# KMS-TEAM/vi_slam

Measured on AMD Instinct MI355X. Metric: frames/sec ORB extract+match, higher is better.
Workload: dtype u8; 1 GPU; kitti00_mono_1241x376_n1000; nfeatures=1000, nlevels=8, contexts_in_flight=4, distinct_frames=32, match=SearchForInitialization(prev frame) window 100

## Files before the change

### vi_slam_amd/csrc/vslam_host.cpp

```cpp
#include "vslam_host.h"
#include "vslam_undistort.h"
#include "vslam_frustum.h"
#include "vslam_kb8.h"
#include "vslam_two_view.h"
#include "vslam_matchdev.h"

#include <algorithm>
#include <climits>
#include <cmath>
#include <cstdlib>
#include <cstring>

namespace vslam {

static inline int cv_round(float v) { return (int)lrintf(v); }
static inline int cv_round(double v) { return (int)lrint(v); }
static inline int cv_floor(float v) {
    int i = (int)v;
    return i - (i > v);
}
static inline int cv_ceil(float v) {
    int i = (int)v;
    return i + (i < v);
}
static inline int16_t sat_short(float v) {
    int iv = cv_round(v);
    return (int16_t)std::min(std::max(iv, (int)SHRT_MIN), (int)SHRT_MAX);
}

void build_tables(int nfeatures, float scaleFactorF, int nlevels, ExtractorTables& t) {
    const double scaleFactor = scaleFactorF;
    t.nlevels = nlevels;
    t.scale.assign(nlevels, 1.0f);
    t.sigma2.assign(nlevels, 1.0f);
    for (int i = 1; i < nlevels; i++) {
        t.scale[i] = (float)(t.scale[i - 1] * scaleFactor);
        t.sigma2[i] = t.scale[i] * t.scale[i];
    }
// ... 585 lines not shown
        P.nIni[l] = nIni;
        P.hX[l] = (float)W / nIni;
        P.selOff[l] = selOff;
        const int cap_l = std::max(P.N[l] + 3, 4 * nIni) + 1;
        selOff += cap_l;
        maxNodes = std::max(maxNodes, cap_l);
        maxNodes = std::max(maxNodes, (cell_first[l + 1] - cell_first[l] + 1 + 3) / 4);
        if (nIni > 64) fits = false;
    }
    P.selStride = selOff;
    P.maxNodes = (maxNodes + 15) & ~15;
    const size_t nb = (node_bytes(P.maxNodes) + 15) & ~(size_t)15;
    int maxcells = 0;
    for (int l = 0; l < L; l++) {
        const int W = lw[l] - 2 * VSLAM_FAST_BORDER, H = P.H[l], nIni = P.nIni[l];
        int D = 1;
        while ((nIni << (2 * D)) < P.N[l]) D++;
        D += 1;
        if (forced_depth >= 0) D = forced_depth;
        D = std::max(1, std::min(D, 11));
        while (D > 1 && (((long long)nIni << (2 * D)) > 16384 || nb + 2 * (((size_t)nIni << (2 * D)) + 1) * 4 + 16 > budget))
            D--;
        P.fineD[l] = D;
        maxcells = std::max(maxcells, nIni << (2 * D));
        std::vector<uint32_t> xs, ys;
        build_oct_lut(W, H, D, xs, ys);
        P.lutOff[l] = (int32_t)P.lut.size();
        P.lutW[l] = (int32_t)xs.size();
        P.lut.insert(P.lut.end(), xs.begin(), xs.end());
        P.lut.insert(P.lut.end(), ys.begin(), ys.end());
    }
    P.fineLdsOff = (int32_t)nb;
    P.fineLdsBytes = (int32_t)(2 * ((size_t)maxcells + 1) * 4 + 16);
    P.fits = fits && nb + (size_t)P.fineLdsBytes <= 160 * 1024 && node_bytes(P.maxNodes) <= 150 * 1024;
}

void build_oct_lut(int W, int H, int D, std::vector<uint32_t>& xs, std::vector<uint32_t>& ys) {
    const int nIni = (int)std::round((float)W / (float)H);
    const float hX = (float)W / (float)nIni;
    xs.assign((size_t)W + 1, 0u);
    ys.assign((size_t)H + 1, 0u);
    for (int x = 0; x <= W; x++) {
        int b = (int)((float)x / hX);
        b = std::min(b, nIni - 1);
        int x0 = (int)(hX * (float)b), x1 = (int)(hX * (float)(b + 1));
        uint32_t code = 0;
        for (int d = 0; d < D; d++) {
            const int mx = x0 + ((x1 - x0 + 1) >> 1);
            const int q = x < mx ? 0 : 1;
            code = (code << 2) | (uint32_t)q;
            if (q) x0 = mx; else x1 = mx;
        }
        xs[x] = ((uint32_t)b << (2 * D)) | code;
    }
    for (int y = 0; y <= H; y++) {
        int y0 = 0, y1 = H;
        uint32_t code = 0;
        for (int d = 0; d < D; d++) {
            const int my = y0 + ((y1 - y0 + 1) >> 1);
            const int q = y < my ? 0 : 1;
            code = (code << 2) | ((uint32_t)q << 1);
            if (q) y0 = my; else y1 = my;
        }
        ys[y] = code;
    }
}

// ... 489 lines not shown
                cur[p] = t.in ? 1 : 0;
            }
            score = vslam_tv::report_score(score);
            if (scores) scores[it] = score;
            const vslam_tv::Best was = best;
            best = vslam_tv::best_take(best, score, it);
            if (best.index != was.index && mask && used) memcpy(mask, cur.data(), (size_t)used);
        }
        (model ? R.best_f : R.best_h) = best.index;
        (model ? R.score_f : R.score_h) = best.index >= 0 ? best.score : 0.0f;
    }
    return err ? VSLAM_ERR_INVALID : n > cap ? VSLAM_ERR_UNSUPPORTED : VSLAM_OK;
}

uint64_t vslamh_layout(uint64_t align, const uint64_t* sizes, int n, uint64_t* off) {
    std::vector<size_t> s(sizes, sizes + n), o(n);
    const size_t total = vslam::layout_parts((size_t)align, s.data(), n, o.data());
    for (int i = 0; i < n; i++) off[i] = o[i];
    return total;
}

int vslamh_oct_lut_check(int W, int H, int D) {
    std::vector<uint32_t> xs, ys;
    vslam::build_oct_lut(W, H, D, xs, ys);
    int bad = 0;
    for (int y = 0; y <= H; y++)
        for (int x = 0; x <= W; x++) bad += (xs[x] | ys[y]) != vslam::oct_key_path(x, y, W, H, D);
    return bad;
}
unsigned vslamh_oct_key_path(int x, int y, int W, int H, int depth) { return vslam::oct_key_path(x, y, W, H, depth); }

int vslamh_keypoint_capacity(const int* quota, const int* lw, const int* lh, int nlevels, int nfeatures) {
    return vslam::keypoint_capacity(quota, lw, lh, nlevels, nfeatures);
}

int vslamh_oct_plan(const int* quota, const int* lw, const int* lh, const int* cell_first, int nlevels, int forced_depth,
                    int budget, int node_per, int node_fixed, int32_t* ctx6, int32_t* lvl4) {
    vslam::OctPlan P;
    vslam::plan_octree(quota, lw, lh, cell_first, nlevels, forced_depth, (size_t)budget,
                       [=](int n) { return (size_t)n * node_per + node_fixed; }, P);
    int bad = 0;
    for (int l = 0; l < nlevels; l++) {
        const int W = P.lutW[l] - 1, H = P.H[l];
        const uint32_t *xs = P.lut.data() + P.lutOff[l], *ys = xs + P.lutW[l];
        for (int y = 0; y <= H; y++)
            for (int x = 0; x <= W; x++) bad += (xs[x] | ys[y]) != vslam::oct_key_path(x, y, W, H, P.fineD[l]);
        const int32_t o[4] = {P.nIni[l], P.selOff[l], P.fineD[l], P.lutW[l]};
        memcpy(lvl4 + 4 * l, o, sizeof(o));
    }
    const int32_t c[6] = {P.maxNodes, P.selStride, P.fineLdsOff, P.fineLdsBytes, P.fits, bad};
    memcpy(ctx6, c, sizeof(c));
    return 0;
}

int vslamh_band_tables(const uint16_t* cells5, int ncells, int nlevels, int max_cells, int max_width, uint32_t* words4,
                       int cap_bands, uint8_t* classes, int cap_class_bytes, int32_t* info5) {
    static_assert(sizeof(vslam::HostCell) == 10 && sizeof(vslam::BandWords) == 16, "rows of five u16 / four u32");
    const vslam::HostCell* c = (const vslam::HostCell*)cells5;
    std::vector<vslam::HostBand> b;
    vslam::build_bands(std::vector<vslam::HostCell>(c, c + ncells), max_cells, max_width, b);
    vslam::BandTables T;
    vslam::pack_bands(b, nlevels, T);
    if ((int)b.size() > cap_bands || (int)T.classes.size() > cap_class_bytes) return -1;
    memcpy(words4, T.bands.data(), T.bands.size() * sizeof(vslam::BandWords));
    memcpy(classes, T.classes.data(), T.classes.size());
    const int32_t o[5] = {(int32_t)(T.classes.size() / 272), T.max_wh, T.max_iw, T.max_cells, T.ok};
// ... 350 lines not shown
```

### vi_slam_amd/csrc/vslam_init_kernel.hip

```cpp
#include "vslam_kernels.h"
#include "vslam_wave.h"
#include "vslam_matchdev.h"

#define SI_TH_LOW 50
#define SI_QPB_MAX 32

struct SiCand {
    float x, y, angle;
    uint16_t cell;
    uint16_t idx;
};
struct SiCandL {
    float x, y;
    uint32_t c;
    uint16_t cell;
    uint16_t idx;
};
struct SiQuery {
    float px, py, angle;
    uint32_t idx;
};

__host__ __device__ inline size_t si_pair_bytes(int max_c2, int M) {
    return 16 + (size_t)max_c2 * (sizeof(SiCand) + sizeof(SiQuery) + 4 * (size_t)M);
}

__global__ void __launch_bounds__(256)
k_si_topm(InitJobs jobs, int cap, SiBounds bnd, int window, int max_c2, int M, uint8_t* scratch, int SI_QPB) {
    extern __shared__ __align__(16) uint8_t sism[];
    SiCandL* cand = (SiCandL*)sism;
    uint32_t* wkeys = (uint32_t*)(cand + max_c2);
    SiCandL* tmpc = (SiCandL*)wkeys;
    __shared__ SiQuery s_q[SI_QPB_MAX];
    __shared__ int s_wcnt[4];
    __shared__ int s_col[SI_GRID_COLS + 1];
// ... 208 lines not shown
    return true;
}

#ifndef SIR_NT
#define SIR_NT 256
#endif
#define SIR_PEND 1u
#define SIR_ACC 2u
#define SIR_SCAN 4u
template <int MAXM>
__global__ void __launch_bounds__(SIR_NT)
k_si_replay(InitJobs jobs, int cap, SiBounds bnd, int window, float nnratio, int checkOri,
            int32_t* matches_out , float* prev_out ,
            int32_t* nmatch_out , int max_c2, int M, const uint8_t* scratch, int* fallbacks, int keys_lds_bytes) {
    extern __shared__ __align__(16) uint8_t sism[];
    const InitJob jb = jobs.job[blockIdx.x];
    const int tid = threadIdx.x, lane = tid & 63;
    const int n1 = min(*jb.cnt1, cap);
    const uint8_t* sp = scratch + (size_t)blockIdx.x * si_pair_bytes(max_c2, M);
    const int32_t* hdr = (const int32_t*)sp;
    const SiCand* gcand = (const SiCand*)(sp + 16);
    const SiQuery* gqry = (const SiQuery*)(gcand + max_c2);
    const uint32_t* topm = (const uint32_t*)(gqry + max_c2);
    const int c1 = hdr[0], c2 = hdr[1];
    uint4* slotlog = (uint4*)sism;
    int32_t* lister0 = (int32_t*)(slotlog + max_c2);
    int32_t* lister1 = lister0 + max_c2;
    uint32_t* kfirst = (uint32_t*)(lister1 + max_c2);
    uint32_t* ksecond = kfirst + max_c2;
    uint32_t* alog = ksecond + max_c2;
    int32_t* m12 = (int32_t*)(alog + max_c2);
    uint8_t* qstate = (uint8_t*)(m12 + cap);
    uint8_t* rotBin = qstate + max_c2;
    uint32_t* keys_lds = (uint32_t*)(sism + (((size_t)max_c2 * 37 + (size_t)cap * 5 + 15) & ~(size_t)15));
    const bool keys_in_lds = (size_t)c1 * M * 4 <= (size_t)keys_lds_bytes;
    const uint32_t* keysrc = keys_in_lds ? keys_lds : topm;
    if (keys_in_lds)
        for (int i = tid; i < c1 * M; i += SIR_NT) keys_lds[i] = topm[i];
    __shared__ int s_hist[VSLAM_HISTO_LENGTH];
    __shared__ int s_minpend[2], s_minwild[2], s_scanq, s_nlog, s_cnt;

    int32_t* mo = matches_out + (size_t)blockIdx.x * cap;
    float* po = prev_out + (size_t)blockIdx.x * cap * 2;
    const SiGridInv inv = si_grid_inv(bnd);
    const float r = (float)window;

    for (int c = tid; c < c2; c += SIR_NT) {
        slotlog[c] = make_uint4(0xFFFFFFFFu, 0xFFFFFFFFu, 0xFFFFFFFFu, 0xFFFFFFFFu);
        lister0[c] = 0x7FFFFFFF;
        lister1[c] = 0x7FFFFFFF;
    }
    for (int q = tid; q < c1; q += SIR_NT) qstate[q] = (uint8_t)SIR_PEND;
    for (int i = tid; i < n1; i += SIR_NT) {
        m12[i] = -1;
        rotBin[i] = 255;
    }
    if (tid < VSLAM_HISTO_LENGTH) s_hist[tid] = 0;
    if (tid == 0) {
        s_minpend[0] = s_minpend[1] = 0x7FFFFFFF;
        s_minwild[0] = s_minwild[1] = 0x7FFFFFFF;
        s_scanq = -1;
        s_nlog = 0;
        s_cnt = 0;
    }
    __syncthreads();

    int nfb = 0, nrounds = 0;
    for (int par = 0;; par ^= 1) {
        int32_t* lister = par ? lister1 : lister0;
        if (tid == 0) s_scanq = -1;
        for (int q = tid; q < c1; q += SIR_NT) {
            if (!(qstate[q] & SIR_PEND)) continue;
            uint32_t key[MAXM];
#pragma unroll
            for (int j = 0; j < MAXM; j++) key[j] = j < M ? keysrc[(size_t)q * M + j] : 0xFFFFFFFFu;
            int nvalid = 0;
            uint32_t gBest = 0xFFFFFFFFu, k2 = 0xFFFFFFFFu, klast = 0u;
#pragma unroll
            for (int j = 0; j < MAXM; j++) {
                if (j < M && key[j] != 0xFFFFFFFFu) {
                    nvalid++;
                    klast = key[j];
                    const uint32_t slot = si_key_index(key[j]), d = si_key_dist(key[j]);
                    if (!(sir_od_eff(slotlog[slot], (uint32_t)q) <= d)) {
                        if (d <= SI_TH_LOW) atomicMin(&lister[slot], q);
                        if (gBest == 0xFFFFFFFFu) gBest = key[j];
                        else if (k2 == 0xFFFFFFFFu) k2 = key[j];
                    }
                }
            }
            const bool full = nvalid == M;
            const uint32_t dlast = si_key_dist(klast);
            const bool wild = full && dlast <= SI_TH_LOW;
            bool accept = false, scan = false;
            if (gBest == 0xFFFFFFFFu) {
                scan = wild;
            } else if (si_key_dist(gBest) <= SI_TH_LOW) {
                uint32_t bestDist2 = k2 == 0xFFFFFFFFu ? 0x7FFFFFFFu : si_key_dist(k2);
                if (k2 == 0xFFFFFFFFu && full) {
                    if ((float)(int)si_key_dist(gBest) < __fmul_rn((float)(int)dlast, nnratio)) bestDist2 = dlast;
                    else scan = true;
                }
                if (!scan) accept = (float)(int)si_key_dist(gBest) < __fmul_rn((float)(int)bestDist2, nnratio);
            }
            kfirst[q] = gBest;
            ksecond[q] = k2;
// ... 91 lines not shown
            const int i = i0 + u * SIR_NT;
            m[u] = i < n1 ? m12[i] : -1;
        }
#pragma unroll
        for (int u = 0; u < 4; u++) {
            const int i = i0 + u * SIR_NT;
            o[u] = make_float2(0.0f, 0.0f);
            if (i < n1) {
                if (m[u] >= 0) o[u] = make_float2(jb.k2[m[u]].x, jb.k2[m[u]].y);
                else if (jb.prev) o[u] = make_float2(jb.prev[2 * i], jb.prev[2 * i + 1]);
                else o[u] = make_float2(jb.k1[i].x, jb.k1[i].y);
            }
        }
#pragma unroll
        for (int u = 0; u < 4; u++) {
            const int i = i0 + u * SIR_NT;
            if (i < n1) {
                mo[i] = m[u];
                po[2 * i] = o[u].x;
                po[2 * i + 1] = o[u].y;
                cnt += m[u] >= 0;
            }
        }
    }
#pragma unroll
    for (int o = 32; o > 0; o >>= 1) cnt += __shfl_xor(cnt, o, 64);
    if (lane == 0 && cnt) atomicAdd(&s_cnt, cnt);
    __syncthreads();
    if (tid == 0) nmatch_out[blockIdx.x] = hdr[2] ? -1 : s_cnt;
}

size_t vk_search_init_scratch_bytes(int npairs, int max_c2, int M) { return (size_t)npairs * si_pair_bytes(max_c2, M); }

static size_t si_topm_lds(int max_c2) { return (size_t)max_c2 * (sizeof(SiCand) + 4 * 4); }
static size_t si_replay_keys_lds(int max_c2, int M) {
    const size_t want = (size_t)max_c2 * M * 4;
    return want <= (64u << 10) ? want : 0;
}
static size_t si_replay_lds(int cap, int max_c2, int M = 0) {
    return (((size_t)max_c2 * 37 + (size_t)cap * 5 + 15) & ~(size_t)15) + si_replay_keys_lds(max_c2, M) + 16;
}

size_t vk_search_init_lds(int cap, int max_c2) { return std::max(si_topm_lds(max_c2), si_replay_lds(cap, max_c2)); }

int vk_search_init_set_max_lds(size_t bytes) {
    int rc = (int)hipFuncSetAttribute((const void*)k_si_topm, hipFuncAttributeMaxDynamicSharedMemorySize, (int)bytes);
    if (rc) return rc;
    rc = (int)hipFuncSetAttribute((const void*)k_si_replay<8>, hipFuncAttributeMaxDynamicSharedMemorySize, (int)bytes);
    if (rc) return rc;
    return (int)hipFuncSetAttribute((const void*)k_si_replay<SI_MAX_M>, hipFuncAttributeMaxDynamicSharedMemorySize, (int)bytes);
}

void vk_search_init(hipStream_t st, const InitJobs& jobs, int npairs, int cap, const SiBounds& bounds, int window,
                    float nnratio, int checkOri, int32_t* matches_out, float* prev_out, int32_t* nmatch_out,
                    int max_c2, int M, uint8_t* scratch, int* fallbacks, const vslam_tuning& T) {
    if (npairs <= 0) return;
    const int qv = T.si_queries_per_block;
    const int qpb = (qv == 8 || qv == 16 || qv == 32) ? qv : 16;
    const int chunks = (max_c2 + qpb - 1) / qpb;
    hipLaunchKernelGGL(k_si_topm, dim3(chunks, npairs), dim3(256), si_topm_lds(max_c2), st, jobs, cap, bounds,
                       window, max_c2, M, scratch, qpb);
    int keys_lds = (int)si_replay_keys_lds(max_c2, M);
    if (si_replay_lds(cap, max_c2, M) > (150u << 10)) keys_lds = 0;
    const size_t rlds = keys_lds ? si_replay_lds(cap, max_c2, M) : si_replay_lds(cap, max_c2);
    if (M <= 8)
        hipLaunchKernelGGL(k_si_replay<8>, dim3(npairs), dim3(SIR_NT), rlds, st, jobs, cap, bounds,
                           window, nnratio, checkOri, matches_out, prev_out, nmatch_out, max_c2, M, scratch, fallbacks, keys_lds);
    else
        hipLaunchKernelGGL(k_si_replay<SI_MAX_M>, dim3(npairs), dim3(SIR_NT), rlds, st, jobs, cap, bounds,
                           window, nnratio, checkOri, matches_out, prev_out, nmatch_out, max_c2, M, scratch, fallbacks, keys_lds);
}
```

### vi_slam_amd/csrc/vslam_octree_kernel.hip

```cpp
#include "vslam_kernels.h"

#include <mutex>

#ifndef O4BATCH
#define O4BATCH 8
#endif
typedef unsigned long long u64;

struct ONode {
    int16_t x0, y0, x1, y1;
    uint32_t begin;
    uint32_t cf;
};
#define ND_NOMORE(nd) ((nd).cf & 1u)

#define FB 21
#define FMASK ((1ull << FB) - 1)
__device__ __forceinline__ unsigned long long onehot(int q) { return q < 3 ? 1ull << (FB * q) : 0ull; }
__device__ __forceinline__ uint32_t fld(unsigned long long v, int q) { return (uint32_t)((v >> (FB * q)) & FMASK); }
__device__ __forceinline__ uint32_t nchildren(unsigned long long c, uint32_t count) {
    const uint32_t c0 = fld(c, 0), c1 = fld(c, 1), c2 = fld(c, 2);
    return (c0 != 0) + (c1 != 0) + (c2 != 0) + (count - c0 - c1 - c2 != 0);
}

template <typename T, int NT>
__device__ __forceinline__ T block_excl_scan(T v, T* s_wave, T* total) {
    const int tid = threadIdx.x, lane = tid & 63, wv = tid >> 6;
    T inc = v;
#pragma unroll
    for (int o = 1; o < 64; o <<= 1) {
        const T t = __shfl_up(inc, o, 64);
        if (lane >= o) inc += t;
    }
// ... 24 lines not shown
        const int mx = x0 + ((x1 - x0 + 1) >> 1), my = y0 + ((y1 - y0 + 1) >> 1);
        const int qx = x < mx ? 0 : 1, qy = y < my ? 0 : 1;
        code = (code << 2) | (uint32_t)qx | ((uint32_t)qy << 1);
        if (qx) x0 = mx; else x1 = mx;
        if (qy) y0 = my; else y1 = my;
    }
    return ((uint32_t)b << (2 * depth)) | code;
}

__device__ __forceinline__ uint32_t wave_incl_add(uint32_t v) {
#pragma unroll
    for (int o = 1; o < 64; o <<= 1) {
        const uint32_t t = __shfl_up(v, o, 64);
        if ((int)(threadIdx.x & 63) >= o) v += t;
    }
    return v;
}

__device__ __forceinline__ u64 deep_child_counts(const uint2* sorted, const uint32_t* PS, uint32_t path, int depth, int D,
                                                 float hX, int nIni, int Hh) {
    u64 c = 0ull;
    const uint32_t f = path >> (2 * (depth - D));
    for (uint32_t j = PS[f]; j < PS[f + 1]; j++) {
        const uint32_t kp = oct_key_path(sorted[j].x, hX, nIni, Hh, depth + 1);
        if ((kp >> 2) == path) c += onehot((int)(kp & 3u));
    }
    return c;
}

#define OCT_BEST(key, pos) ((((key) >> 24) << 20) | (0xFFFFFu - (uint32_t)(pos)))
#define OCT_BEST_POS(b) (0xFFFFFu - ((b) & 0xFFFFFu))

template <int OTV>
__global__ void __launch_bounds__(OTV)
k_octree_v4(const uint8_t* __restrict__ cand_region, size_t cand_stride, int ncells, OctParams P, uint32_t* keys_a,
            uint2* sorted_a, size_t pts_stride, uint32_t* sel_xyr, int32_t* sel_cnt, int32_t* err_flag,
            int32_t* deep_flags) {
    extern __shared__ __align__(16) uint8_t osm[];
    const int MAXN = P.maxNodes;
    ONode* cur = (ONode*)osm;
    ONode* nxt = cur + MAXN;
    uint32_t* Kq = (uint32_t*)(nxt + MAXN);
    u64* Cnt = (u64*)(nxt + MAXN) + MAXN;
    uint16_t* cb = (uint16_t*)(Cnt + MAXN);
    uint16_t* newIdx = cb + MAXN;
    uint16_t* prank = newIdx + MAXN;
    uint16_t* ordv = prank + MAXN;
    __shared__ uint32_t s_w32[OTV / 64];
    __shared__ int s_size, s_M, s_nexp, s_cut, s_deep;

    const int tid = threadIdx.x, lane = tid & 63, wv = tid >> 6;
    const int level = blockIdx.y, slot = blockIdx.x;
    const int N = P.N[level];
    const uint32_t* hdr = (const uint32_t*)(cand_region + (size_t)slot * cand_stride);
    const CellOut* cout = (const CellOut*)(hdr + 2);
    const uint32_t* cand = (const uint32_t*)(cout + ncells);
    uint32_t* pa = keys_a + (size_t)slot * pts_stride;
    uint2* sorted = sorted_a + (size_t)slot * pts_stride;
    uint32_t* out = sel_xyr + (size_t)slot * P.selStride + P.selOff[level];
    int32_t* ocnt = sel_cnt + slot * VSLAM_MAX_LEVELS + level;
    if (tid == 0) {
        deep_flags[slot * VSLAM_MAX_LEVELS + level] = 0;
        s_deep = 0;
    }
#ifdef VSLAM_OCT_STAMPS
    int dbgn3 = 0;
    unsigned long long* DBG3 = (unsigned long long*)P.dbg;
#ifndef VSLAM_OCT_STAMP_LEVEL
#define VSLAM_OCT_STAMP_LEVEL 0
#endif
#define STAMP3() do { if (DBG3 && tid == 0 && level == VSLAM_OCT_STAMP_LEVEL && slot == 0 && dbgn3 < 60) DBG3[dbgn3++] = __builtin_amdgcn_s_memrealtime(); } while (0)
#else
#define STAMP3() do { } while (0)
#endif
    STAMP3();

    const int c0 = P.cellFirst[level], c1 = P.cellFirst[level + 1];
    uint32_t off0 = 0;
    if (c0 > 0) {
        uint32_t before = 0;
        for (int c = tid; c < c0; c += OTV) before += cout[c].count;
        uint32_t tot;
        block_excl_scan<uint32_t, OTV>(before, s_w32, &tot);
        off0 = tot;
    }
    const int ncl = c1 - c0, K = (ncl + OTV - 1) / OTV;
    uint32_t mine = 0;
    for (int k = 0; k < K; k++) {
        const int c = c0 + tid * K + k;
        if (c < c1) mine += cout[c].count;
    }
    uint32_t ntot;
    uint32_t woff = block_excl_scan<uint32_t, OTV>(mine, s_w32, &ntot);
    const int n = (int)ntot;
    if (off0 + ntot > (uint32_t)P.ptsCap || n >= (1 << 20) || hdr[1] != 0) {
        if (tid == 0) {
// ... 91 lines not shown
            const uint32_t inc = wave_incl_add(h);
            if (c < cells) PS[c] = carry + inc - h;
            carry += (uint32_t)__builtin_amdgcn_readlane((int)inc, 63);
        }
        if (lane == 0) s_w32[wv] = carry;
        __syncthreads();
        uint32_t wo = 0;
        for (int k = 0; k < wv; k++) wo += s_w32[k];
        if (wo)
            for (int t = wv * tpw; t < t1; t++) {
                const int c = t * 64 + lane;
                if (c < cells) PS[c] += wo;
            }
        if (tid == 0) PS[cells] = (uint32_t)n;
    }
    __syncthreads();
    STAMP3();

    if (tid == 0) {
        int li = 0;
        for (int b = 0; b < nIni; b++) {
            const uint32_t cb0 = PS[(b + 1) << (2 * D)] - PS[b << (2 * D)];
            if (cb0) {
                ONode nd;
                nd.x0 = (int16_t)(int)__fmul_rn(hX, (float)b);
                nd.x1 = (int16_t)(int)__fmul_rn(hX, (float)(b + 1));
                nd.y0 = 0;
                nd.y1 = (int16_t)Hh;
                nd.begin = (uint32_t)b;
                nd.cf = (cb0 << 1) | (cb0 == 1 ? 1u : 0u);
                cur[li++] = nd;
            }
        }
        s_size = li;
    }
    __syncthreads();
    STAMP3();

    int phase = 1;
    bool haveSorted = false;
    const int KN = (MAXN + OTV - 1) / OTV;
    for (int iter = 0; iter < P.maxIter; iter++) {
        const int size0 = s_size;
        for (int k = 0; k < KN; k++) {
            const int v = tid * KN + k;
            if (v < size0) {
                const ONode nd = cur[v];
                u64 c = 0ull;
                uint32_t kq = 0u;
                if (!ND_NOMORE(nd)) {
                    const int depth = ND4_DEPTH(nd);
                    const uint32_t path = nd.begin;
                    if (depth < D) {
                        const uint32_t cb0 = path << (2 * (D - depth)), q4 = 1u << (2 * (D - depth - 1));
                        const uint32_t p0 = PS[cb0], p1 = PS[cb0 + q4], p2 = PS[cb0 + 2 * q4], p3 = PS[cb0 + 3 * q4];
                        c = (u64)(p1 - p0) | ((u64)(p2 - p1) << FB) | ((u64)(p3 - p2) << (2 * FB));
                    } else {
                        s_deep = 1;
                        if (haveSorted) c = deep_child_counts(sorted, PS, path, depth, D, hX, nIni, Hh);
                    }
                    kq = (ND4_COUNT(nd) << 12) | (uint32_t)(4095 - v);
                }
                Cnt[v] = c;
                Kq[v] = kq;
            }
        }
        if (tid < 4 && size0 + tid < ((size0 + 3) & ~3)) Kq[size0 + tid] = 0u;
        __syncthreads();
        if (s_deep && !haveSorted) {
            for (int i = tid; i < cells; i += OTV) Bst[i] = 0u;
            __syncthreads();
            for (int base = tid; base < n; base += O4BATCH * OTV) {
                uint32_t kk[O4BATCH], ff[O4BATCH];
#pragma unroll
                for (int j = 0; j < O4BATCH; j++) kk[j] = base + j * OTV < n ? pa[base + j * OTV] : 0u;
#pragma unroll
                for (int j = 0; j < O4BATCH; j++) ff[j] = base + j * OTV < n ? xs[kk[j] & 0xFFF] | ys[(kk[j] >> 12) & 0xFFF] : 0u;
#pragma unroll
                for (int j = 0; j < O4BATCH; j++) {
                    const int i = base + j * OTV;
                    if (i < n) sorted[PS[ff[j]] + atomicAdd(&Bst[ff[j]], 1u)] = make_uint2(kk[j], (uint32_t)i);
                }
            }
            haveSorted = true;
            __syncthreads();
            for (int k = 0; k < KN; k++) {
                const int v = tid * KN + k;
                if (v < size0) {
                    const ONode nd = cur[v];
                    if (!ND_NOMORE(nd) && ND4_DEPTH(nd) >= D)
                        Cnt[v] = deep_child_counts(sorted, PS, nd.begin, ND4_DEPTH(nd), D, hX, nIni, Hh);
                }
            }
            __syncthreads();
        }
        uint32_t nexp_mine = 0;
        for (int k = 0; k < KN; k++) {
            const int v = tid * KN + k;
            if (v < size0 && !ND_NOMORE(cur[v])) nexp_mine++;
        }
        uint32_t nexp;
        uint32_t rbase = block_excl_scan<uint32_t, OTV>(nexp_mine, s_w32, &nexp);
// ... 7 lines not shown
                    rbase++;
                }
            }
        } else {
            const uint4* K4 = (const uint4*)Kq;
            const int n4 = (size0 + 3) >> 2;
            for (int k = 0; k < KN; k++) {
                const int v = tid * KN + k;
                if (v < size0 && !ND_NOMORE(cur[v])) {
                    const uint32_t kv = Kq[v];
                    uint32_t r = 0;
#pragma unroll 4
                    for (int u = 0; u < n4; u++) {
                        const uint4 q = K4[u];
                        r += (q.x > kv) + (q.y > kv) + (q.z > kv) + (q.w > kv);
                    }
                    prank[v] = (uint16_t)r;
                    ordv[r] = (uint16_t)v;
                }
            }
        }
        __syncthreads();
        const int KE = ((int)nexp + OTV - 1) / OTV;
        uint32_t chl = 0;
        for (int k = 0; k < KE; k++) {
            const int r = tid * KE + k;
            if (r < (int)nexp) {
                const int v = ordv[r];
                chl += nchildren(Cnt[v], ND4_COUNT(cur[v]));
            }
        }
        uint32_t chtot;
        uint32_t chbase = block_excl_scan<uint32_t, OTV>(chl, s_w32, &chtot);
        if (tid == 0) s_cut = (int)nexp;
        __syncthreads();
        {
            uint32_t cb_run = chbase;
            for (int k = 0; k < KE; k++) {
                const int r = tid * KE + k;
                if (r < (int)nexp) {
                    const int v = ordv[r];
                    const uint32_t nch = nchildren(Cnt[v], ND4_COUNT(cur[v]));
                    if (phase == 2 && size0 + (int)cb_run - r >= N) atomicMin(&s_cut, r);
                    cb[v] = (uint16_t)cb_run;
                    cb_run += nch;
                }
            }
        }
        __syncthreads();
        const int ncut = s_cut;
        if (tid == 0) {
            int M;
            if (ncut >= (int)nexp) M = (int)chtot;
            else M = cb[ordv[ncut]];
            s_M = M;
            s_size = size0 + M - ncut;
            s_nexp = 0;
        }
        __syncthreads();
        const int M = s_M;
        uint32_t sv = 0;
        for (int k = 0; k < KN; k++) {
            const int v = tid * KN + k;
            if (v < size0) {
                const bool processed = !ND_NOMORE(cur[v]) && prank[v] < ncut;
                if (!processed) sv++;
            }
        }
        uint32_t svtot;
        uint32_t svbase = block_excl_scan<uint32_t, OTV>(sv, s_w32, &svtot);
        int nexp_children = 0;
        for (int k = 0; k < KN; k++) {
            const int v = tid * KN + k;
            if (v >= size0) continue;
            const ONode nd = cur[v];
            const bool processed = !ND_NOMORE(nd) && prank[v] < ncut;
            if (!processed) {
                nxt[M + svbase] = nd;
                svbase++;
            } else {
                const u64 c = Cnt[v];
                const int mx = nd.x0 + ((nd.x1 - nd.x0 + 1) >> 1), my = nd.y0 + ((nd.y1 - nd.y0 + 1) >> 1);
                const uint32_t depth1 = (uint32_t)ND4_DEPTH(nd) + 1u;
                int kq = 0;
                const int first = M - 1 - (int)cb[v];
                const uint32_t c3 = ND4_COUNT(nd) - fld(c, 0) - fld(c, 1) - fld(c, 2);
                for (int q = 0; q < 4; q++) {
                    const uint32_t cq = q < 3 ? fld(c, q) : c3;
                    if (!cq) continue;
                    ONode ch;
                    ch.x0 = (q & 1) ? (int16_t)mx : nd.x0;
                    ch.x1 = (q & 1) ? nd.x1 : (int16_t)mx;
                    ch.y0 = (q & 2) ? (int16_t)my : nd.y0;
                    ch.y1 = (q & 2) ? nd.y1 : (int16_t)my;
                    ch.begin = (nd.begin << 2) | (uint32_t)q;
                    ch.cf = (depth1 << 28) | (cq << 1) | (cq == 1 ? 1u : 0u);
                    nxt[first - kq] = ch;
                    if (cq > 1) nexp_children++;
                    kq++;
                }
            }
        }
        if (nexp_children) atomicAdd(&s_nexp, nexp_children);
        __syncthreads();
        { ONode* t = cur; cur = nxt; nxt = t; }
        const int size = s_size, nToExpand = s_nexp;
        __syncthreads();
        STAMP3();
        if (size >= N || size == size0) break;
        if (phase == 1 && size + nToExpand * 3 > N) phase = 2;
    }

    STAMP3();
    const int size = s_size;
    if (!haveSorted) {
        uint32_t* win = (uint32_t*)nxt;
        for (int v0 = 0; v0 < size; v0 += OTV / 4) {
            const int v = v0 + (tid >> 2), sub = tid & 3;
            uint32_t best = 0u;
            if (v < size) {
                const ONode nd = cur[v];
                const int sh = 2 * (D - ND4_DEPTH(nd));
                const uint32_t lo = nd.begin << sh, hi = (nd.begin + 1u) << sh;
                for (uint32_t j = lo + (uint32_t)sub; j < hi; j += 4) best = max(best, Bst[j]);
            }
            best = max(best, (uint32_t)__shfl_xor((int)best, 1, 64));
            best = max(best, (uint32_t)__shfl_xor((int)best, 2, 64));
            if (v < size && sub == 0) win[v] = OCT_BEST_POS(best);
        }
        __syncthreads();
        for (int v = tid; v < size; v += OTV) out[v] = pa[win[v]];
    } else {
        for (int v0 = 0; v0 < size; v0 += OTV / 4) {
            const int v = v0 + (tid >> 2), sub = tid & 3;
            u64 best = 0ull;
            uint32_t bkey = 0u;
            if (v < size) {
                const ONode nd = cur[v];
                const int depth = ND4_DEPTH(nd);
                const uint32_t path = nd.begin;
                if (depth <= D) {
                    const uint32_t lo = PS[path << (2 * (D - depth))], hi = PS[(path + 1u) << (2 * (D - depth))];
                    for (uint32_t j0 = lo + (uint32_t)sub; j0 < hi; j0 += 16) {
                        uint2 r[4];
#pragma unroll
                        for (int u = 0; u < 4; u++) r[u] = j0 + 4 * u < hi ? sorted[j0 + 4 * u] : make_uint2(0u, 0xFFFFFFFFu);
#pragma unroll
// ... 8 lines not shown
                } else {
                    const uint32_t f = path >> (2 * (depth - D));
                    for (uint32_t j = PS[f] + (uint32_t)sub; j < PS[f + 1]; j += 4) {
                        const uint2 r = sorted[j];
                        if (oct_key_path(r.x, hX, nIni, Hh, depth) == path) {
                            const u64 a = ((u64)(r.x >> 24) << 32) | (u64)(0xFFFFFFFFu - r.y);
                            if (a >= best) {
                                best = a;
                                bkey = r.x;
                            }
                        }
                    }
                }
            }
#pragma unroll
            for (int o = 1; o < 4; o <<= 1) {
                const u64 ob = __shfl_xor(best, o, 64);
                const uint32_t ok = __shfl_xor(bkey, o, 64);
                if (ob > best) {
                    best = ob;
                    bkey = ok;
                }
            }
            if (v < size && sub == 0) out[v] = bkey;
        }
    }
#ifdef VSLAM_OCT_STAMPS
    __syncthreads();
    STAMP3();
    if (DBG3 && tid == 0 && level == VSLAM_OCT_STAMP_LEVEL && slot == 0) DBG3[63] = dbgn3;
#endif
    if (tid == 0) {
        *ocnt = size;
        if (s_deep) deep_flags[slot * VSLAM_MAX_LEVELS + level] = 1;
    }
}

#define AO_T 256
__global__ void __launch_bounds__(AO_T)
k_assign_out(OctParams P, PyramidGeom g, uint32_t* sel_xyr, int32_t* sel_cnt,
             int lap0, int lap1, SelKp* sel, int32_t* slot_counts , int cap,
             int32_t* err_flag, const int32_t* deep_flags) {
    __shared__ uint32_t s_w32[AO_T / 64];
    __shared__ int s_lvl_off[VSLAM_MAX_LEVELS + 1];
    const int tid = threadIdx.x, slot = blockIdx.x;
    const int L = g.nlevels;
    uint32_t redo_mask = 0;
    if (deep_flags && tid == 0)
        for (int lv = 0; lv < L; lv++) redo_mask |= deep_flags[slot * VSLAM_MAX_LEVELS + lv] ? 1u << lv : 0u;
    if (tid == 0) {
        int acc = 0;
        for (int l = 0; l < L; l++) {
            s_lvl_off[l] = acc;
            acc += sel_cnt[slot * VSLAM_MAX_LEVELS + l];
        }
        s_lvl_off[L] = acc;
    }
    __syncthreads();
    const int nk = s_lvl_off[L];
    if (nk > cap) {
        if (tid == 0) {
            atomicOr(err_flag, 2);
            slot_counts[slot * 4] = 0;
            slot_counts[slot * 4 + 1] = 0;
            slot_counts[slot * 4 + 2] = (int32_t)redo_mask;
        }
        return;
// ... 8 lines not shown
        const uint32_t p = base[P.selOff[l] + (i - s_lvl_off[l])];
        float px = (float)((int)(p & 0xFFF) + VSLAM_BORDER);
        if (l) px = __fmul_rn(px, g.lv[l].scale);
        lapc += (px >= (float)lap0 && px <= (float)lap1) ? 1u : 0u;
    }
    uint32_t laptot;
    uint32_t lapbefore = block_excl_scan<uint32_t, AO_T>(lapc, s_w32, &laptot);
    l = 0;
    for (int i = i0; i < i1; i++) {
        while (i >= s_lvl_off[l + 1]) l++;
        const uint32_t p = base[P.selOff[l] + (i - s_lvl_off[l])];
        const int lx = (int)(p & 0xFFF) + VSLAM_BORDER, ly = (int)((p >> 12) & 0xFFF) + VSLAM_BORDER;
        float px = (float)lx;
        if (l) px = __fmul_rn(px, g.lv[l].scale);
        const bool inlap = px >= (float)lap0 && px <= (float)lap1;
        SelKp k;
        k.x = (uint16_t)lx;
        k.y = (uint16_t)ly;
        k.level = (uint8_t)l;
        k.slot = (uint8_t)slot;
        k.response = (uint8_t)(p >> 24);
        k.pad = 0;
        k.out = inlap ? (uint32_t)(nk - 1 - (int)lapbefore) : (uint32_t)(i - (int)lapbefore);
        if (inlap) lapbefore++;
        sel[(size_t)slot * cap + i] = k;
    }
    if (tid == 0) {
        slot_counts[slot * 4] = nk;
        slot_counts[slot * 4 + 1] = nk - (int)laptot;
        slot_counts[slot * 4 + 2] = (int32_t)redo_mask;
    }
}

size_t vk_octree_lds_bytes(int maxNodes) { return (size_t)maxNodes * (16 + 16 + 8 + 8 + 2 + 2 + 2 + 2) + 64; }

void vk_octree(hipStream_t st, const uint8_t* cand_region, size_t cand_stride, int ncells, const OctParams& P,
               uint32_t* keys_a, void* sorted_a, size_t pts_stride,
               uint32_t* sel_xyr, int32_t* sel_cnt, int32_t* err_flag, int nlevels, int nslots, int32_t* deep_flags,
               int regkeys , int threads ) {
    const dim3 grid(nslots, nlevels);
    const bool rk = regkeys < 0 ? nslots <= 2 : regkeys == 1;
    const size_t lds = (size_t)P.fineLdsOff + (size_t)P.fineLdsBytes;
    const int th = rk ? 1024 : (threads == 256 || threads == 512) ? threads : 1024;
#define OCT4_LAUNCH(TH)                                                                                          \
    hipLaunchKernelGGL((k_octree_v4<TH>), grid, dim3(TH), lds, st, cand_region, cand_stride, ncells, P, keys_a, \
                       (uint2*)sorted_a, pts_stride, sel_xyr, sel_cnt, err_flag, deep_flags)
    if (th == 256) OCT4_LAUNCH(256);
    else if (th == 512) OCT4_LAUNCH(512);
    else OCT4_LAUNCH(1024);
#undef OCT4_LAUNCH
}

void vk_assign_out(hipStream_t st, const OctParams& P, const PyramidGeom& g, uint32_t* sel_xyr, int32_t* sel_cnt, int lap0,
                   int lap1, SelKp* sel, int32_t* slot_counts, int cap, int32_t* err_flag, int nslots,
                   const int32_t* deep_flags) {
    hipLaunchKernelGGL(k_assign_out, dim3(nslots), dim3(AO_T), 0, st, P, g, sel_xyr, sel_cnt, lap0, lap1, sel,
                       slot_counts, cap, err_flag, deep_flags);
}

int vk_octree_set_max_lds(size_t bytes) {
    static std::mutex mu;
    static size_t have_dev[64] = {0};
    std::lock_guard<std::mutex> lk(mu);
    int dev = 0;
    if (hipGetDevice(&dev) != hipSuccess || dev < 0 || dev >= 64) return (int)hipErrorInvalidDevice;
    size_t& have = have_dev[dev];
    if (bytes <= have) return 0;
// ... 9 lines not shown
```

Before: 211,200 frames/s.

## Shrink octree and search-init LDS footprints and pin octree occupancy

Adds a shared LDS layout header that packs the octree node arrays without gaps, drops the unused newIdx array, and gathers per-block statics into one struct. The octree kernel now requests eight waves per EU, and the search-init replay kernel caches only as many query keys in LDS as fit a size budget, reading the rest from global memory. The aim is to lower per-block LDS and register use so more blocks stay resident. The risks are register spills from the occupancy attribute and extra global loads for uncached keys.

```diff
diff --git a/vi_slam_amd/csrc/vslam_host.cpp b/vi_slam_amd/csrc/vslam_host.cpp
--- a/vi_slam_amd/csrc/vslam_host.cpp
+++ b/vi_slam_amd/csrc/vslam_host.cpp
@@ -4,6 +4,7 @@
 #include "vslam_kb8.h"
 #include "vslam_two_view.h"
 #include "vslam_matchdev.h"
+#include "vslam_lds_layout.h"
 
 #include <algorithm>
 #include <climits>
@@ -655,7 +656,8 @@
     }
     P.fineLdsOff = (int32_t)nb;
     P.fineLdsBytes = (int32_t)(2 * ((size_t)maxcells + 1) * 4 + 16);
-    P.fits = fits && nb + (size_t)P.fineLdsBytes <= 160 * 1024 && node_bytes(P.maxNodes) <= 150 * 1024;
+    const size_t judged = std::max(node_bytes(P.maxNodes), (size_t)P.maxNodes * VSLAM_OCT_PLACEMENT_NODE_BYTES + VSLAM_OCT_FIXED_BYTES);
+    P.fits = fits && nb + (size_t)P.fineLdsBytes <= 160 * 1024 && judged <= 150 * 1024;
 }
 
 void build_oct_lut(int W, int H, int D, std::vector<uint32_t>& xs, std::vector<uint32_t>& ys) {
@@ -1211,6 +1213,16 @@
 
 int vslamh_keypoint_capacity(const int* quota, const int* lw, const int* lh, int nlevels, int nfeatures) {
     return vslam::keypoint_capacity(quota, lw, lh, nlevels, nfeatures);
+}
+
+int vslamh_lds_layout(int cap, int max_c2, int M, int32_t* oct8, int32_t* sir4) {
+    const int32_t o[8] = {VSLAM_OCT_NODE_BYTES, VSLAM_OCT_FIXED_BYTES, VSLAM_OCT_BORROW_BYTES, vslam_oct_static_lds(256),
+                          vslam_oct_static_lds(512), vslam_oct_static_lds(1024), VSLAM_FAST_HOLE_LDS, VSLAM_FAST_HOLE_VGPRS};
+    memcpy(oct8, o, sizeof(o));
+    const int32_t r[4] = {(int32_t)vslam_sir_lds_bytes(cap, max_c2, M), (int32_t)vslam_sir_keys_bytes(cap, max_c2, M),
+                          vslam_sir_static_lds(), (int32_t)vslam_sir_lds_bytes(cap, max_c2, 0)};
+    memcpy(sir4, r, sizeof(r));
+    return 0;
 }
 
 int vslamh_oct_plan(const int* quota, const int* lw, const int* lh, const int* cell_first, int nlevels, int forced_depth,
diff --git a/vi_slam_amd/csrc/vslam_init_kernel.hip b/vi_slam_amd/csrc/vslam_init_kernel.hip
--- a/vi_slam_amd/csrc/vslam_init_kernel.hip
+++ b/vi_slam_amd/csrc/vslam_init_kernel.hip
@@ -1,6 +1,7 @@
 #include "vslam_kernels.h"
 #include "vslam_wave.h"
 #include "vslam_matchdev.h"
+#include "vslam_lds_layout.h"
 
 #define SI_TH_LOW 50
 #define SI_QPB_MAX 32
@@ -275,13 +276,16 @@
     int32_t* m12 = (int32_t*)(alog + max_c2);
     uint8_t* qstate = (uint8_t*)(m12 + cap);
     uint8_t* rotBin = qstate + max_c2;
-    uint32_t* keys_lds = (uint32_t*)(sism + (((size_t)max_c2 * 37 + (size_t)cap * 5 + 15) & ~(size_t)15));
-    const bool keys_in_lds = (size_t)c1 * M * 4 <= (size_t)keys_lds_bytes;
-    const uint32_t* keysrc = keys_in_lds ? keys_lds : topm;
-    if (keys_in_lds)
-        for (int i = tid; i < c1 * M; i += SIR_NT) keys_lds[i] = topm[i];
-    __shared__ int s_hist[VSLAM_HISTO_LENGTH];
-    __shared__ int s_minpend[2], s_minwild[2], s_scanq, s_nlog, s_cnt;
+    uint32_t* keys_lds = (uint32_t*)(sism + vslam_sir_state_bytes(cap, max_c2));
+    const int qcached = min(c1, keys_lds_bytes / (M * 4));
+    for (int i = tid; i < qcached * M; i += SIR_NT) keys_lds[i] = topm[i];
+    __shared__ VslamSirStatic s_st;
+    int* const s_hist = s_st.hist;
+    int* const s_minpend = s_st.minpend;
+    int* const s_minwild = s_st.minwild;
+    int& s_scanq = s_st.scanq;
+    int& s_nlog = s_st.nlog;
+    int& s_cnt = s_st.cnt;
 
     int32_t* mo = matches_out + (size_t)blockIdx.x * cap;
     float* po = prev_out + (size_t)blockIdx.x * cap * 2;
@@ -315,6 +319,7 @@
         for (int q = tid; q < c1; q += SIR_NT) {
             if (!(qstate[q] & SIR_PEND)) continue;
             uint32_t key[MAXM];
+            const uint32_t* keysrc = q < qcached ? keys_lds : topm;
 #pragma unroll
             for (int j = 0; j < MAXM; j++) key[j] = j < M ? keysrc[(size_t)q * M + j] : 0xFFFFFFFFu;
             int nvalid = 0;
@@ -472,14 +477,10 @@
 
 size_t vk_search_init_scratch_bytes(int npairs, int max_c2, int M) { return (size_t)npairs * si_pair_bytes(max_c2, M); }
 
+static_assert(VSLAM_SIR_HISTO == VSLAM_HISTO_LENGTH, "vslam_lds_layout.h sizes k_si_replay's histogram");
 static size_t si_topm_lds(int max_c2) { return (size_t)max_c2 * (sizeof(SiCand) + 4 * 4); }
-static size_t si_replay_keys_lds(int max_c2, int M) {
-    const size_t want = (size_t)max_c2 * M * 4;
-    return want <= (64u << 10) ? want : 0;
-}
-static size_t si_replay_lds(int cap, int max_c2, int M = 0) {
-    return (((size_t)max_c2 * 37 + (size_t)cap * 5 + 15) & ~(size_t)15) + si_replay_keys_lds(max_c2, M) + 16;
-}
+static size_t si_replay_keys_lds(int cap, int max_c2, int M) { return vslam_sir_keys_bytes(cap, max_c2, M); }
+static size_t si_replay_lds(int cap, int max_c2, int M = 0) { return vslam_sir_lds_bytes(cap, max_c2, M); }
 
 size_t vk_search_init_lds(int cap, int max_c2) { return std::max(si_topm_lds(max_c2), si_replay_lds(cap, max_c2)); }
 
@@ -500,7 +501,7 @@
     const int chunks = (max_c2 + qpb - 1) / qpb;
     hipLaunchKernelGGL(k_si_topm, dim3(chunks, npairs), dim3(256), si_topm_lds(max_c2), st, jobs, cap, bounds,
                        window, max_c2, M, scratch, qpb);
-    int keys_lds = (int)si_replay_keys_lds(max_c2, M);
+    int keys_lds = (int)si_replay_keys_lds(cap, max_c2, M);
     if (si_replay_lds(cap, max_c2, M) > (150u << 10)) keys_lds = 0;
     const size_t rlds = keys_lds ? si_replay_lds(cap, max_c2, M) : si_replay_lds(cap, max_c2);
     if (M <= 8)
diff --git a/vi_slam_amd/csrc/vslam_lds_layout.h b/vi_slam_amd/csrc/vslam_lds_layout.h
--- /dev/null
+++ b/vi_slam_amd/csrc/vslam_lds_layout.h
@@ -0,0 +1,47 @@
+#pragma once
+#include <cstddef>
+#include <cstdint>
+
+#define VSLAM_FAST_HOLE_LDS (20480 - 64 + 16)
+#define VSLAM_FAST_HOLE_VGPRS 64
+
+#define VSLAM_OCT_NODE_BYTES 50
+#define VSLAM_OCT_FIXED_BYTES 64
+#define VSLAM_OCT_PLACEMENT_NODE_BYTES 56
+#define VSLAM_OCT_OFF_NXT 16
+#define VSLAM_OCT_OFF_KQ 32
+#define VSLAM_OCT_OFF_CNT 36
+#define VSLAM_OCT_OFF_CB 44
+#define VSLAM_OCT_OFF_PRANK 46
+#define VSLAM_OCT_OFF_ORDV 48
+#define VSLAM_OCT_BORROW_BYTES (VSLAM_OCT_NODE_BYTES - VSLAM_OCT_OFF_NXT)
+
+inline size_t vslam_oct_node_lds_bytes(int maxNodes) { return (size_t)maxNodes * VSLAM_OCT_NODE_BYTES + VSLAM_OCT_FIXED_BYTES; }
+
+template <int OTV>
+struct VslamOctStatic {
+    uint32_t w32[OTV / 64];
+    int size, M, nexp, cut, deep;
+};
+inline int vslam_oct_static_lds(int threads) {
+    const size_t s = threads == 256 ? sizeof(VslamOctStatic<256>) : threads == 512 ? sizeof(VslamOctStatic<512>) : sizeof(VslamOctStatic<1024>);
+    return (int)((s + 15) & ~(size_t)15);
+}
+
+#define VSLAM_SIR_HISTO 30
+struct VslamSirStatic {
+    int hist[VSLAM_SIR_HISTO];
+    int minpend[2], minwild[2], scanq, nlog, cnt;
+};
+inline int vslam_sir_static_lds() { return (int)((sizeof(VslamSirStatic) + 15) & ~(size_t)15); }
+constexpr size_t vslam_sir_state_bytes(int cap, int max_c2) { return ((size_t)max_c2 * 37 + (size_t)cap * 5 + 15) & ~(size_t)15; }
+inline size_t vslam_sir_keys_bytes(int cap, int max_c2, int M) {
+    const size_t want = (size_t)max_c2 * M * 4;
+    if (M <= 0 || want > (64u << 10)) return 0;
+    const size_t fixed = vslam_sir_state_bytes(cap, max_c2) + 16 + (size_t)vslam_sir_static_lds();
+    if (fixed + want <= VSLAM_FAST_HOLE_LDS || fixed >= VSLAM_FAST_HOLE_LDS) return want;
+    return (VSLAM_FAST_HOLE_LDS - fixed) / ((size_t)M * 4) * ((size_t)M * 4);
+}
+inline size_t vslam_sir_lds_bytes(int cap, int max_c2, int M) {
+    return vslam_sir_state_bytes(cap, max_c2) + vslam_sir_keys_bytes(cap, max_c2, M) + 16;
+}
diff --git a/vi_slam_amd/csrc/vslam_octree_kernel.hip b/vi_slam_amd/csrc/vslam_octree_kernel.hip
--- a/vi_slam_amd/csrc/vslam_octree_kernel.hip
+++ b/vi_slam_amd/csrc/vslam_octree_kernel.hip
@@ -1,4 +1,5 @@
 #include "vslam_kernels.h"
+#include "vslam_lds_layout.h"
 
 #include <mutex>
 
@@ -89,22 +90,21 @@
 #define OCT_BEST_POS(b) (0xFFFFFu - ((b) & 0xFFFFFu))
 
 template <int OTV>
-__global__ void __launch_bounds__(OTV)
+__global__ void __launch_bounds__(OTV) __attribute__((amdgpu_waves_per_eu(8, 8)))
 k_octree_v4(const uint8_t* __restrict__ cand_region, size_t cand_stride, int ncells, OctParams P, uint32_t* keys_a,
             uint2* sorted_a, size_t pts_stride, uint32_t* sel_xyr, int32_t* sel_cnt, int32_t* err_flag,
             int32_t* deep_flags) {
     extern __shared__ __align__(16) uint8_t osm[];
     const int MAXN = P.maxNodes;
     ONode* cur = (ONode*)osm;
-    ONode* nxt = cur + MAXN;
-    uint32_t* Kq = (uint32_t*)(nxt + MAXN);
-    u64* Cnt = (u64*)(nxt + MAXN) + MAXN;
-    uint16_t* cb = (uint16_t*)(Cnt + MAXN);
-    uint16_t* newIdx = cb + MAXN;
-    uint16_t* prank = newIdx + MAXN;
-    uint16_t* ordv = prank + MAXN;
-    __shared__ uint32_t s_w32[OTV / 64];
-    __shared__ int s_size, s_M, s_nexp, s_cut, s_deep;
+    ONode* nxt = (ONode*)(osm + (size_t)MAXN * VSLAM_OCT_OFF_NXT);
+    uint32_t* Kq = (uint32_t*)(osm + (size_t)MAXN * VSLAM_OCT_OFF_KQ);
+    u64* Cnt = (u64*)(osm + (size_t)MAXN * VSLAM_OCT_OFF_CNT);
+    uint16_t* cb = (uint16_t*)(osm + (size_t)MAXN * VSLAM_OCT_OFF_CB);
+    uint16_t* prank = (uint16_t*)(osm + (size_t)MAXN * VSLAM_OCT_OFF_PRANK);
+    uint16_t* ordv = (uint16_t*)(osm + (size_t)MAXN * VSLAM_OCT_OFF_ORDV);
+    __shared__ VslamOctStatic<OTV> s_st;
+    uint32_t* const s_w32 = s_st.w32;
 
     const int tid = threadIdx.x, lane = tid & 63, wv = tid >> 6;
     const int level = blockIdx.y, slot = blockIdx.x;
@@ -118,7 +118,7 @@
     int32_t* ocnt = sel_cnt + slot * VSLAM_MAX_LEVELS + level;
     if (tid == 0) {
         deep_flags[slot * VSLAM_MAX_LEVELS + level] = 0;
-        s_deep = 0;
+        s_st.deep = 0;
     }
 #ifdef VSLAM_OCT_STAMPS
     int dbgn3 = 0;
@@ -276,7 +276,7 @@
                 cur[li++] = nd;
             }
         }
-        s_size = li;
+        s_st.size = li;
     }
     __syncthreads();
     STAMP3();
@@ -285,7 +285,7 @@
     bool haveSorted = false;
     const int KN = (MAXN + OTV - 1) / OTV;
     for (int iter = 0; iter < P.maxIter; iter++) {
-        const int size0 = s_size;
+        const int size0 = s_st.size;
         for (int k = 0; k < KN; k++) {
             const int v = tid * KN + k;
             if (v < size0) {
@@ -300,7 +300,7 @@
                         const uint32_t p0 = PS[cb0], p1 = PS[cb0 + q4], p2 = PS[cb0 + 2 * q4], p3 = PS[cb0 + 3 * q4];
                         c = (u64)(p1 - p0) | ((u64)(p2 - p1) << FB) | ((u64)(p3 - p2) << (2 * FB));
                     } else {
-                        s_deep = 1;
+                        s_st.deep = 1;
                         if (haveSorted) c = deep_child_counts(sorted, PS, path, depth, D, hX, nIni, Hh);
                     }
                     kq = (ND4_COUNT(nd) << 12) | (uint32_t)(4095 - v);
@@ -311,7 +311,7 @@
         }
         if (tid < 4 && size0 + tid < ((size0 + 3) & ~3)) Kq[size0 + tid] = 0u;
         __syncthreads();
-        if (s_deep && !haveSorted) {
+        if (s_st.deep && !haveSorted) {
             for (int i = tid; i < cells; i += OTV) Bst[i] = 0u;
             __syncthreads();
             for (int base = tid; base < n; base += O4BATCH * OTV) {
@@ -385,7 +385,7 @@
         }
         uint32_t chtot;
         uint32_t chbase = block_excl_scan<uint32_t, OTV>(chl, s_w32, &chtot);
-        if (tid == 0) s_cut = (int)nexp;
+        if (tid == 0) s_st.cut = (int)nexp;
         __syncthreads();
         {
             uint32_t cb_run = chbase;
@@ -394,24 +394,24 @@
                 if (r < (int)nexp) {
                     const int v = ordv[r];
                     const uint32_t nch = nchildren(Cnt[v], ND4_COUNT(cur[v]));
-                    if (phase == 2 && size0 + (int)cb_run - r >= N) atomicMin(&s_cut, r);
+                    if (phase == 2 && size0 + (int)cb_run - r >= N) atomicMin(&s_st.cut, r);
                     cb[v] = (uint16_t)cb_run;
                     cb_run += nch;
                 }
             }
         }
         __syncthreads();
-        const int ncut = s_cut;
+        const int ncut = s_st.cut;
         if (tid == 0) {
             int M;
             if (ncut >= (int)nexp) M = (int)chtot;
             else M = cb[ordv[ncut]];
-            s_M = M;
-            s_size = size0 + M - ncut;
-            s_nexp = 0;
-        }
-        __syncthreads();
-        const int M = s_M;
+            s_st.M = M;
+            s_st.size = size0 + M - ncut;
+            s_st.nexp = 0;
+        }
+        __syncthreads();
+        const int M = s_st.M;
         uint32_t sv = 0;
         for (int k = 0; k < KN; k++) {
             const int v = tid * KN + k;
@@ -454,10 +454,10 @@
                 }
             }
         }
-        if (nexp_children) atomicAdd(&s_nexp, nexp_children);
+        if (nexp_children) atomicAdd(&s_st.nexp, nexp_children);
         __syncthreads();
         { ONode* t = cur; cur = nxt; nxt = t; }
-        const int size = s_size, nToExpand = s_nexp;
+        const int size = s_st.size, nToExpand = s_st.nexp;
         __syncthreads();
         STAMP3();
         if (size >= N || size == size0) break;
@@ -465,7 +465,7 @@
     }
 
     STAMP3();
-    const int size = s_size;
+    const int size = s_st.size;
     if (!haveSorted) {
         uint32_t* win = (uint32_t*)nxt;
         for (int v0 = 0; v0 < size; v0 += OTV / 4) {
@@ -540,7 +540,7 @@
 #endif
     if (tid == 0) {
         *ocnt = size;
-        if (s_deep) deep_flags[slot * VSLAM_MAX_LEVELS + level] = 1;
+        if (s_st.deep) deep_flags[slot * VSLAM_MAX_LEVELS + level] = 1;
     }
 }
 
@@ -615,7 +615,12 @@
     }
 }
 
-size_t vk_octree_lds_bytes(int maxNodes) { return (size_t)maxNodes * (16 + 16 + 8 + 8 + 2 + 2 + 2 + 2) + 64; }
+static_assert(sizeof(ONode) == VSLAM_OCT_OFF_NXT && VSLAM_OCT_OFF_KQ == 2 * sizeof(ONode) && VSLAM_OCT_OFF_KQ % 16 == 0 &&
+                  VSLAM_OCT_OFF_CNT == VSLAM_OCT_OFF_KQ + 4 && VSLAM_OCT_OFF_CNT % 4 == 0 && VSLAM_OCT_OFF_CB == VSLAM_OCT_OFF_CNT + 8 &&
+                  VSLAM_OCT_OFF_PRANK == VSLAM_OCT_OFF_CB + 2 && VSLAM_OCT_OFF_ORDV == VSLAM_OCT_OFF_PRANK + 2 &&
+                  VSLAM_OCT_NODE_BYTES == VSLAM_OCT_OFF_ORDV + 2,
+              "the node arrays follow each other without gaps; maxNodes % 16 == 0 aligns Kq to 16 and Cnt to 8 bytes");
+size_t vk_octree_lds_bytes(int maxNodes) { return vslam_oct_node_lds_bytes(maxNodes); }
 
 void vk_octree(hipStream_t st, const uint8_t* cand_region, size_t cand_stride, int ncells, const OctParams& P,
                uint32_t* keys_a, void* sorted_a, size_t pts_stride,
```

New measurement: 211,300 frames/s, median of 3. About the same (+0.0%).
